# HKU-BAL/Clair3-RNA

Hardware: NVIDIA B200
Metric: candidate sites/sec (tensor+inference) (higher is better)
Workload: dtype int32 pileup + fp16/fp32-accumulate network

## Files before the change

clair3_rna_b200/build.py:

```python
import os
import subprocess
import sys

HERE = os.path.dirname(os.path.abspath(__file__))
CSRC = os.path.join(HERE, "csrc")
LIB = os.path.join(HERE, "libc3r_b200.so")
SOURCES = ["c3r_abi.cu", "bam_io.cpp", "decode.cpp", "fasta_io.cpp"]
HEADERS = ["scan.cuh", "pileup.cuh", "nn_fp32.cuh", "nn_tc.cuh", "nn_lstm2f.cuh", "tc_ptx.cuh", os.path.join("..", "..", "include", "c3r_b200.h")]
NVCC_FLAGS = ["-gencode", "arch=compute_100a,code=sm_100a", "-lineinfo", "-O3", "-std=c++17",
              "-Xcompiler", "-fPIC", "-shared", "-lcuda", "-lz", "-lpthread"]


def needs_build():
    if not os.path.exists(LIB):
        return True
    t = os.path.getmtime(LIB)
    return any(os.path.getmtime(os.path.join(CSRC, f)) > t for f in SOURCES + HEADERS)


def build(force=False, verbose=False):
    if not force and not needs_build():
        return LIB
    nvcc = os.environ.get("NVCC", "/usr/local/cuda/bin/nvcc")
    cmd = [nvcc] + NVCC_FLAGS + (["-Xptxas", "-v"] if verbose else []) + ["-o", LIB] + SOURCES
    out = subprocess.run(cmd, cwd=CSRC, stdout=subprocess.PIPE, stderr=subprocess.STDOUT, text=True)
    if out.returncode != 0:
        sys.stderr.write(out.stdout)
        raise RuntimeError("nvcc failed building libc3r_b200.so")
    if verbose:
        print(out.stdout)
    return LIB


if __name__ == "__main__":
    print(build(force="--force" in sys.argv, verbose="-v" in sys.argv))
```

clair3_rna_b200/csrc/nn_lstm2f.cuh:

```cuda
#pragma once

namespace c3r {

namespace ptx {
__device__ __forceinline__ void bulk_g2s_mcast(uint32_t dst, const void* src, uint32_t bytes, uint32_t bar, uint16_t mask) {
    asm volatile(
        "cp.async.bulk.shared::cluster.global.mbarrier::complete_tx::bytes.multicast::cluster [%0], [%1], %2, [%3], %4;"
        ::"r"(dst), "l"(src), "r"(bytes), "r"(bar), "h"(mask) : "memory");
}
}

constexpr int L2F_CH = 5;
constexpr int L2F_IMG = 8192;
constexpr int L2F_STAGES = 6;
constexpr int L2F_SLOT = 2 * L2F_IMG;
constexpr int L2F_LAST = 64 * 48 * 2;
constexpr int L2F_CHUNK_BYTES = 10 * L2F_IMG + L2F_LAST;
constexpr int L2F_STREAM_BYTES = L2F_CH * L2F_CHUNK_BYTES;
constexpr int L2F_NS = 4;
constexpr int L2F_GATE_WARPS = 16;
constexpr int L2F_THREADS = 128 + 32 * L2F_GATE_WARPS;
constexpr int L2F_AH = TC_TILE * U2 * 2;
constexpr int L2F_XB = TC_IMG * 2;
constexpr int L2F_OFF_X = 2 * L2F_AH;
// ... 173 lines not shown
            if (n_steps > 0)
                for (int kb = 0; kb < 4; ++kb) ptx::mbar_wait(b_xfree + 8 * kb, (n_steps - 1) & 1, a.err, 331);
        }
    } else if (warp == 2) {
        if (lane == 0) {
            const uint8_t* wsrc = a.wstream + ((size_t)dir * 2 + hr) * L2F_STREAM_BYTES;
            uint32_t wslot = 0, wph = 0, it = 0;
            long long pw[1] = {0};
            for (uint32_t g = 0; g < n_steps; ++g) {
                uint32_t off = 0;
                for (int cs = 0; cs < CH * L2F_STAGES; ++cs, ++it) {
                    const uint32_t bytes = (cs % L2F_STAGES) == L2F_STAGES - 1 ? L2F_LAST : L2F_SLOT;
                    L2F_WAIT(b_we + 8 * wslot, wph ^ 1, 340, 0);
                    ptx::mbar_arrive_expect_tx(b_wf + 8 * wslot, bytes);
                    if (NP == 1) ptx::bulk_g2s(s_W + wslot * L2F_SLOT, wsrc + off, bytes, b_wf + 8 * wslot);
                    else if (it % NP == pr) ptx::bulk_g2s_mcast(s_W + wslot * L2F_SLOT, wsrc + off, bytes, b_wf + 8 * wslot, mask_half);
                    off += bytes;
                    if (++wslot == L2F_NS) { wslot = 0; wph ^= 1; }
                }
            }
            if (PROF && pf) a.prof[8] = pw[0];
            const uint32_t total = n_steps * CH * L2F_STAGES;
            for (uint32_t k = total > (uint32_t)L2F_NS ? total - L2F_NS : 0; k < total; ++k)
                ptx::mbar_wait(b_we + 8 * (k % L2F_NS), (k / L2F_NS) & 1, a.err, 341);
        }
    } else if (warp == 3) {
        if (lane == 0 && hr == 1) {
            uint32_t wslot = 0, wph = 0;
            for (uint32_t g = 0; g < n_steps; ++g)
                for (int c = 0; c < CH; ++c)
                    for (int s = 0; s < L2F_STAGES; ++s) {
                        if (c == 0 && s < 4) {
                            ptx::mbar_wait(b_xf + 8 * s, g & 1, a.err, 350);
                            ptx::mbar_arrive_cluster_relaxed(b_xf + 8 * s, leader);
                        }
                        ptx::mbar_wait(b_wf + 8 * wslot, wph, a.err, 351);
                        ptx::mbar_arrive_cluster_relaxed(b_wf + 8 * wslot, leader);
                        if (++wslot == L2F_NS) { wslot = 0; wph ^= 1; }
                    }
        }
    } else {
        const int gw = warp - 4;
        const int q = warp & 3;
        const int sub = gw >> 2;
        const int row = q * 32 + lane;
        const uint32_t lane_addr = (uint32_t)(q * 32) << 16;
        uint32_t use = 0;
        const bool pfg = pf && gw == 0;
        long long pw[1] = {0};
        for (uint32_t g = 0; g < n_steps; ++g) {
            const int r = (int)(g / NT), step = (int)(g % NT);
            const int tp = j + r * J;
            const bool valid = tp < n_tile_pairs;
            const int tile = (valid ? tp : n_tile_pairs - 1) * 2 + (int)hr;
            const uint32_t nbuf = (g + 1) & 1;
            const int t = dir == 0 ? step : NT - 1 - step;
            uint8_t* ah = smem + nbuf * L2F_AH;
            __half* hout_t = a.hout + ((size_t)tile * NT + t) * 5 * TC_IMG;
            __half* hout_lo_t = a.hout_lo + ((size_t)tile * NT + t) * 5 * TC_IMG;
#pragma unroll
            for (int c = 0; c < CH; ++c, ++use) {
                const uint32_t slot = use & 1;
                if (PROF && pfg) { const long long t0 = clock64(); ptx::mbar_wait(b_accf + 8 * slot, (use >> 1) & 1, a.err, 308); pw[0] += clock64() - t0; }
                else ptx::mbar_wait(b_accf + 8 * slot, (use >> 1) & 1, a.err, 308);
                ptx::tc_fence_after();
                uint32_t cprev[8];
                uint32_t v[4][8];
#pragma unroll
                for (int gte = 0; gte < 4; ++gte) ptx::tmem_ld8(tmem + lane_addr + slot * 128 + gte * 32 + sub * 8, v[gte]);
                if (step > 0) ptx::tmem_ld8(tmem + lane_addr + C_COL + c * 32 + sub * 8, cprev);
                ptx::tmem_wait_ld();
                ptx::tc_fence_before();
                __syncwarp();
                if (lane == 0) ptx::mbar_arrive(b_acce + 8 * slot);
                uint32_t cnew[8];
                __align__(16) __half hh[8];
                __align__(16) __half hl[8];
#pragma unroll
                for (int u = 0; u < 8; ++u) {
                    const float zi = __uint_as_float(v[0][u]), zf = __uint_as_float(v[1][u]);
                    const float zg = __uint_as_float(v[2][u]), zo = __uint_as_float(v[3][u]);
                    const float cp = step > 0 ? __uint_as_float(cprev[u]) : 0.0f;
                    float cn, hv;
                    lstm_cell(zi, zf, zg, zo, cp, cn, hv);
                    cnew[u] = __float_as_uint(cn);
                    hh[u] = __float2half(hv);
                    hl[u] = __float2half(hv - __half2float(hh[u]));
                }
                ptx::tmem_st8(tmem + lane_addr + C_COL + c * 32 + sub * 8, cnew);
                const uint4 pk = *(const uint4*)hh;
                const int k8 = c * 4 + sub;
                *(uint4*)(ah + (size_t)k8 * (TC_TILE * 16) + row * 16) = pk;
                ptx::tmem_wait_st();
                if (c == CH - 1) {
                    ptx::tc_fence_before();
                    ptx::fence_proxy_async();
                    __syncwarp();
                    if (lane == 0) ptx::mbar_arrive(b_hrdy);
                }
                if (valid) {
                    const int col8 = (dir * U2) / 8 + k8;
                    const size_t oo = (size_t)(col8 / 8) * TC_IMG + (size_t)(col8 % 8) * (TC_TILE * 8) + row * 8;
                    *(uint4*)(hout_t + oo) = pk;
                    if (a.hout_lo) *(uint4*)(hout_lo_t + oo) = *(const uint4*)hl;
                }
            }
        }
        if (PROF && pfg && lane == 0) a.prof[9] = pw[0];
    }
    ptx::tc_fence_before();
    __syncthreads();
    ptx::cluster_sync();
    if (warp == 0) ptx::tmem_dealloc<2>(tmem, 512);
}

inline void lstm2f_pack(std::vector<uint8_t>& out, const float* h, size_t o_w2, size_t o_b2, size_t o_u2) {
    out.assign((size_t)4 * L2F_STREAM_BYTES, 0);
    auto split = [](float w, __half& hi, __half& lo) {
        hi = __float2half(w);
        lo = __float2half(w - __half2float(hi));
    };
    for (int dir = 0; dir < 2; ++dir)
        for (int hr = 0; hr < 2; ++hr) {
            __half* base = (__half*)(out.data() + ((size_t)dir * 2 + hr) * L2F_STREAM_BYTES);
            for (int c = 0; c < L2F_CH; ++c) {
                __half* ch = base + (size_t)c * (L2F_CHUNK_BYTES / 2);
                for (int jj = 0; jj < 64; ++jj) {
                    const int col = hr * 64 + jj, gate = col / 32, ul = col % 32;
                    const int kc = gate * U2 + c * 32 + ul;
                    const float gs = gate == 2 ? 1.0f : 0.5f;
                    for (int kb = 0; kb < 4; ++kb)
                        for (int k = 0; k < 64; ++k) {
                            __half hi, lo;
                            split(gs * h[o_w2 + (size_t)(kb * 64 + k) * 2 * G2 + dir * G2 + kc], hi, lo);
                            ch[(size_t)(2 * kb) * (L2F_IMG / 2) + ((size_t)(k / 8) * 64 * 8 + (size_t)jj * 8 + k % 8)] = hi;
                            ch[(size_t)(2 * kb + 1) * (L2F_IMG / 2) + ((size_t)(k / 8) * 64 * 8 + (size_t)jj * 8 + k % 8)] = lo;
                        }
                    for (int k = 0; k < U2; ++k) {
                        const int s = 8 + k / 64, kk = k % 64;
                        ch[(size_t)s * (L2F_IMG / 2) + ((size_t)(kk / 8) * 64 * 8 + (size_t)jj * 8 + kk % 8)] =
                            __float2half(gs * h[o_u2 + (size_t)dir * U2 * G2 + (size_t)k * G2 + kc]);
                    }
                    __half bh, bl;
                    split(gs * h[o_b2 + dir * G2 + kc], bh, bl);
                    __half* st10 = ch + (size_t)10 * (L2F_IMG / 2);
                    st10[(size_t)(32 / 8) * 64 * 8 + (size_t)jj * 8 + 0] = bh;
                    st10[(size_t)(32 / 8) * 64 * 8 + (size_t)jj * 8 + 1] = bl;
                }
            }
        }
}

template <int NP, bool PROF>
inline cudaError_t launch_lstm2f_np(const Lstm2fArgs& a, int sm_count, cudaStream_t st) {
    static bool attr = false;
    if (!attr) {
        cudaError_t e = cudaFuncSetAttribute(k_lstm2_fused<NP, PROF>, cudaFuncAttributeMaxDynamicSharedMemorySize, L2F_SMEM);
        if (e != cudaSuccess) return e;
        attr = true;
    }
    const int csize = 2 * NP;
    const int tile_pairs = a.n_tiles / 2;
    int per_dir = (tile_pairs + NP - 1) / NP;
    int max_per_dir = sm_count / csize / 2;
    if (NP > 1) {
        cudaLaunchConfig_t q = {};
        q.gridDim = dim3((unsigned)(sm_count / csize * csize)); q.blockDim = dim3(L2F_THREADS); q.dynamicSmemBytes = L2F_SMEM;
        cudaLaunchAttribute qa[1];
        qa[0].id = cudaLaunchAttributeClusterDimension;
        qa[0].val.clusterDim.x = csize; qa[0].val.clusterDim.y = 1; qa[0].val.clusterDim.z = 1;
        q.attrs = qa; q.numAttrs = 1;
        int n_cl = 0;
        if (cudaOccupancyMaxActiveClusters(&n_cl, k_lstm2_fused<NP, PROF>, &q) == cudaSuccess && n_cl > 0 && n_cl / 2 < max_per_dir)
            max_per_dir = n_cl / 2;
    }
    if (max_per_dir < 1) max_per_dir = 1;
    if (per_dir > max_per_dir) per_dir = max_per_dir;
    if (per_dir < 1) per_dir = 1;
    cudaLaunchConfig_t cfg = {};
    cfg.gridDim = dim3((unsigned)(per_dir * 2 * csize));
    cfg.blockDim = dim3(L2F_THREADS);
    cfg.dynamicSmemBytes = L2F_SMEM;
    cfg.stream = st;
    cudaLaunchAttribute at[1];
    at[0].id = cudaLaunchAttributeClusterDimension;
    at[0].val.clusterDim.x = csize; at[0].val.clusterDim.y = 1; at[0].val.clusterDim.z = 1;
    cfg.attrs = at; cfg.numAttrs = 1;
    return cudaLaunchKernelEx(&cfg, k_lstm2_fused<NP, PROF>, a);
}

inline int lstm2f_np() {
    static int v = -1;
    if (v < 0) {
        const char* e = getenv("C3R_LSTM2F_NP");
        v = e ? atoi(e) : 1;
        if (v != 1 && v != 2 && v != 4) v = 1;
    }
    return v;
}

inline cudaError_t launch_lstm2f(const Lstm2fArgs& a, int sm_count, cudaStream_t st) {
    if (a.prof) return launch_lstm2f_np<1, true>(a, sm_count, st);
    switch (lstm2f_np()) {
        case 2: return launch_lstm2f_np<2, false>(a, sm_count, st);
        case 4: return launch_lstm2f_np<4, false>(a, sm_count, st);
        default: return launch_lstm2f_np<1, false>(a, sm_count, st);
    }
}

}
```

clair3_rna_b200/csrc/nn_tc.cuh:

```cuda
#pragma once
#include <cstdint>
#include <cstdlib>
#include <string>
#include <vector>
#include <cuda_runtime.h>
#include <cuda_fp16.h>
#include "nn_fp32.cuh"
#include "tc_ptx.cuh"

namespace c3r {

constexpr int TC_TILE = 128;
constexpr int TC_KB = 64;
constexpr int TC_IMG = TC_TILE * TC_KB;
constexpr int lstm1_kx(int C) { return (3 * C + 2 + 15) / 16 * 16; }
constexpr int LSTM1_KX_MAX = lstm1_kx(30);

struct GemmArgs {
    const __half* A;
    const __half* B;
    const __half* A_lo;
    const __half* B_lo;
    int terms;
    const float* bias;
    float* out;
    int m_tiles, n_tiles, n_kb;
    int ksplit;
    size_t split_stride;
    int* err;
};

constexpr int GEMM_STAGES = 3;
constexpr int GEMM_THREADS = 192;
constexpr int GEMM_STAGE_BYTES = 4 * TC_IMG * 2;
constexpr int GEMM_SMEM = GEMM_STAGES * GEMM_STAGE_BYTES + 1024;

__global__ void __launch_bounds__(GEMM_THREADS, 1) k_gemm_tc(GemmArgs g) {
    extern __shared__ __align__(1024) uint8_t smem[];
    uint64_t* bars = (uint64_t*)(smem + GEMM_STAGES * GEMM_STAGE_BYTES);
    uint32_t* tmem_ptr_s = (uint32_t*)(bars + 12);
    float* bias_s = (float*)(bars + 32);
    const uint32_t s_base = ptx::smem_u32(smem);
    const uint32_t b_full = ptx::smem_u32(bars), b_empty = b_full + 32, b_accf = b_full + 64, b_acce = b_full + 80;
    const int warp = threadIdx.x >> 5, lane = threadIdx.x & 31;
    if (threadIdx.x == 0) {
        for (int i = 0; i < GEMM_STAGES; ++i) { ptx::mbar_init(b_full + 8 * i, 1); ptx::mbar_init(b_empty + 8 * i, 1); }
        for (int i = 0; i < 2; ++i) { ptx::mbar_init(b_accf + 8 * i, 1); ptx::mbar_init(b_acce + 8 * i, 4); }
        ptx::fence_barrier_init();
    }
    if (warp == 1) {
        ptx::tmem_alloc<1>(ptx::smem_u32(tmem_ptr_s), 256);
        ptx::tmem_relinquish<1>();
    }
    ptx::tc_fence_before();
    __syncthreads();
    ptx::tc_fence_after();
    const uint32_t tmem = *tmem_ptr_s;
    const int n_tiles_total = g.m_tiles * g.n_tiles;
    const int ksplit = g.ksplit > 1 ? g.ksplit : 1;
    const int n_items = n_tiles_total * ksplit;
    const uint32_t idesc = ptx::make_idesc_f16(128, 128);

    if (warp == 0) {
        if (lane == 0) {
            uint32_t it = 0;
            for (int item = blockIdx.x; item < n_items; item += gridDim.x) {
                const int tile = item % n_tiles_total, ks = item / n_tiles_total;
                const int m = tile / g.n_tiles, n = tile % g.n_tiles;
                const size_t ao = (size_t)m * g.n_kb * TC_IMG, bo = (size_t)n * g.n_kb * TC_IMG;
                const int kb0 = ks * g.n_kb / ksplit, kb1 = (ks + 1) * g.n_kb / ksplit;
                for (int kb = kb0; kb < kb1; ++kb, ++it) {
                    const uint32_t s = it % GEMM_STAGES, ph = (it / GEMM_STAGES) & 1;
                    const uint32_t dst = s_base + s * GEMM_STAGE_BYTES;
                    ptx::mbar_wait(b_empty + 8 * s, ph ^ 1, g.err, 101);
                    const bool a_lo = g.terms & 2;
                    ptx::mbar_arrive_expect_tx(b_full + 8 * s, a_lo ? GEMM_STAGE_BYTES : GEMM_STAGE_BYTES - TC_IMG * 2);
                    ptx::bulk_g2s(dst, g.A + ao + (size_t)kb * TC_IMG, TC_IMG * 2, b_full + 8 * s);
                    if (a_lo) ptx::bulk_g2s(dst + TC_IMG * 2, g.A_lo + ao + (size_t)kb * TC_IMG, TC_IMG * 2, b_full + 8 * s);
                    ptx::bulk_g2s(dst + 2 * TC_IMG * 2, g.B + bo + (size_t)kb * TC_IMG, TC_IMG * 2, b_full + 8 * s);
                    ptx::bulk_g2s(dst + 3 * TC_IMG * 2, g.B_lo + bo + (size_t)kb * TC_IMG, TC_IMG * 2, b_full + 8 * s);
                }
            }
        }
    } else if (warp == 1) {
        if (lane == 0) {
            uint32_t it = 0, tc = 0;
            for (int item = blockIdx.x; item < n_items; item += gridDim.x, ++tc) {
                const int ks = item / n_tiles_total;
                const int kb0 = ks * g.n_kb / ksplit, kb1 = (ks + 1) * g.n_kb / ksplit;
                const uint32_t slot = tc & 1, aph = (tc >> 1) & 1;
                ptx::mbar_wait(b_acce + 8 * slot, aph ^ 1, g.err, 102);
                ptx::tc_fence_after();
                for (int kb = kb0; kb < kb1; ++kb, ++it) {
                    const uint32_t s = it % GEMM_STAGES, ph = (it / GEMM_STAGES) & 1;
                    ptx::mbar_wait(b_full + 8 * s, ph, g.err, 103);
                    ptx::tc_fence_after();
                    const uint32_t st0 = s_base + s * GEMM_STAGE_BYTES;
#pragma unroll
                    for (int term = 0; term < 3; ++term) {
                        if (!((g.terms >> term) & 1)) continue;
                        const uint32_t sa = st0 + (term == 1 ? TC_IMG * 2 : 0), sb = st0 + (term == 2 ? 3 : 2) * TC_IMG * 2;
#pragma unroll
                        for (int k4 = 0; k4 < TC_KB / 16; ++k4) {
                            const uint64_t da = ptx::make_smem_desc(sa + k4 * 2 * (TC_TILE * 16), TC_TILE * 16, 128);
                            const uint64_t db = ptx::make_smem_desc(sb + k4 * 2 * (TC_TILE * 16), TC_TILE * 16, 128);
                            ptx::mma_f16<1>(tmem + slot * 128, da, db, idesc, (kb > kb0 || term > 0 || k4 > 0) ? 1u : 0u);
                        }
                    }
                    ptx::mma_commit_1(b_empty + 8 * s);
                }
                ptx::mma_commit_1(b_accf + 8 * slot);
            }
        }
    } else {
        const int q = warp & 3;
        const int row = q * 32 + lane;
        uint32_t tc = 0;
        for (int item = blockIdx.x; item < n_items; item += gridDim.x, ++tc) {
            const int tile = item % n_tiles_total, ks = item / n_tiles_total;
            const int m = tile / g.n_tiles, n = tile % g.n_tiles;
            const uint32_t slot = tc & 1, aph = (tc >> 1) & 1;
            ptx::mbar_wait(b_accf + 8 * slot, aph, g.err, 104);
            ptx::tc_fence_after();
            const uint32_t taddr = tmem + ((uint32_t)(q * 32) << 16) + slot * 128;
            asm volatile("bar.sync 1, 128;" ::: "memory");
            bias_s[threadIdx.x - 64] = g.bias[(size_t)n * 128 + (threadIdx.x - 64)];
            asm volatile("bar.sync 1, 128;" ::: "memory");
            const float* bias = bias_s;
#pragma unroll 1
            for (int j = 0; j < 8; ++j) {
                uint32_t v[16];
                ptx::tmem_ld16(taddr + j * 16, v);
                ptx::tmem_wait_ld();
                float* o = g.out + ((size_t)m * 128 + row) * ((size_t)g.n_tiles * 128) + (size_t)n * 128 + j * 16;
                if (ksplit > 1) {
                    float4* o4 = (float4*)(o + (size_t)ks * g.split_stride);
#pragma unroll
                    for (int c = 0; c < 4; ++c)
                        o4[c] = make_float4(__uint_as_float(v[4 * c]), __uint_as_float(v[4 * c + 1]), __uint_as_float(v[4 * c + 2]), __uint_as_float(v[4 * c + 3]));
                } else {
#pragma unroll
                    for (int c = 0; c < 16; ++c) o[c] = seluf_(__uint_as_float(v[c]) + bias[j * 16 + c]);
                }
            }
            ptx::tc_fence_before();
            __syncwarp();
            if (lane == 0) ptx::mbar_arrive(b_acce + 8 * slot);
        }
    }
    ptx::tc_fence_before();
    __syncthreads();
    if (warp == 1) ptx::tmem_dealloc<1>(tmem, 256);
}

template <int CH, int KX>
struct LstmCfg {
    static constexpr int U = CH * 32;
    static constexpr int KT = KX + U;
    static constexpr int B_BYTES = CH * 64 * KT * 2;
    static constexpr int AH_BYTES = TC_TILE * U * 2;
// ... 372 lines not shown
    void* abuf = nullptr;
    size_t abytes = 0;
    int cap_tiles = 0;
    __half* h1[2] = {};
    __half *h2 = nullptr, *h2_lo = nullptr, *xop = nullptr;
    __half* h1_cur = nullptr;
    float *l4 = nullptr, *l4p = nullptr;
    size_t l4_stride = 0;
    __half *l4h = nullptr, *l4h_lo = nullptr;
    float* a5 = nullptr;
    int* err = nullptr;
    long long* trace = nullptr;
    bool attr_set = false;
    struct TcPipe* pipe = nullptr;
};

inline void tc_pipe_release(struct TcPipe* p);
inline void tc_release(TcNet& t) {
    if (t.pipe) tc_pipe_release(t.pipe);
    if (t.wbuf) cudaFree(t.wbuf);
    if (t.abuf) cudaFree(t.abuf);
    if (t.err) cudaFree(t.err);
    if (t.trace) cudaFree(t.trace);
    t = TcNet();
}

inline size_t img_index(int R, int r, int k) { return (size_t)(k / 8) * R * 8 + (size_t)r * 8 + (k % 8); }

inline int tc_build(TcNet& t, const NetF32& net, const float* h, size_t o_w1, size_t o_b1, size_t o_u1, size_t o_w2,
                    size_t o_b2, size_t o_u2, size_t o_k4, size_t o_b4, size_t o_k51, size_t o_b51, size_t o_k52, size_t o_b52,
                    int sm_count, std::string* err) {
    tc_release(t);
    const int C = net.C;
    t.C = C;
    t.KX = lstm1_kx(C);
    t.sm_count = sm_count;
    const int KX = t.KX;
    const int KT1 = KX + U1;
    const size_t n_img1 = (size_t)2 * 2 * 4 * 64 * KT1;
    const size_t n_k4p = (size_t)(L4_IN / TC_KB) * TC_IMG;
    const size_t n_k5p = (size_t)2 * 2 * TC_IMG;
    std::vector<__half> hb(n_img1 + 2 * n_k4p + 2 * n_k5p);
    std::vector<float> fb(DENSE + 2 * DENSE);
    __half* img1 = hb.data();
    __half* k4p = img1 + n_img1;
    __half* k4p_lo = k4p + n_k4p;
    __half* k5p = k4p_lo + n_k4p;
    __half* k5p_lo = k5p + n_k5p;
    auto split = [](float w, __half& hi, __half& lo) {
        hi = __float2half(w);
        lo = __float2half(w - __half2float(hi));
    };
    for (int dir = 0; dir < 2; ++dir)
        for (int rank = 0; rank < 2; ++rank)
            for (int c = 0; c < 4; ++c) {
                __half* im = img1 + ((((size_t)dir * 2 + rank) * 4 + c) * 64) * KT1;
                for (int j = 0; j < 64; ++j) {
                    const int col = rank * 64 + j, gate = col / 32, ul = col % 32;
                    const int kc = gate * U1 + c * 32 + ul;
                    const float gs = gate == 2 ? 1.0f : 0.5f;
                    for (int k = 0; k < KT1; ++k) {
                        __half v = __float2half(0.0f);
                        if (k < 3 * C) {
                            const int ch = k % C;
                            __half hi, lo;
                            split(gs * h[o_w1 + (size_t)ch * 2 * G1 + dir * G1 + kc], hi, lo);
                            v = k >= C && k < 2 * C ? lo : hi;
                        } else if (k == 3 * C || k == 3 * C + 1) {
                            __half hi, lo;
                            split(gs * h[o_b1 + dir * G1 + kc], hi, lo);
                            v = k == 3 * C ? hi : lo;
                        } else if (k >= KX) {
                            v = __float2half(gs * h[o_u1 + (size_t)dir * U1 * G1 + (size_t)(k - KX) * G1 + kc]);
                        }
                        im[img_index(64, j, k)] = v;
                    }
                }
            }
    for (int k = 0; k < L4_IN; ++k)
        for (int j = 0; j < DENSE; ++j)
        {
            const size_t ix = (size_t)(k / TC_KB) * TC_IMG + img_index(128, j, k % TC_KB);
            split(h[o_k4 + (size_t)k * DENSE + j], k4p[ix], k4p_lo[ix]);
        }
    for (int j = 0; j < DENSE; ++j) fb[j] = h[o_b4 + j];
    for (int n = 0; n < 2; ++n)
        for (int k = 0; k < DENSE; ++k)
            for (int j = 0; j < DENSE; ++j) {
                const size_t ix = ((size_t)n * 2 + k / TC_KB) * TC_IMG + img_index(128, j, k % TC_KB);
                split(h[(n == 0 ? o_k51 : o_k52) + (size_t)k * DENSE + j], k5p[ix], k5p_lo[ix]);
            }
    for (int j = 0; j < DENSE; ++j) { fb[DENSE + j] = h[o_b51 + j]; fb[2 * DENSE + j] = h[o_b52 + j]; }

    std::vector<uint8_t> ws;
    lstm2f_pack(ws, h, o_w2, o_b2, o_u2);
    const size_t foff = ((hb.size() * 2 + 255) / 256) * 256;
    const size_t soff = ((foff + fb.size() * 4 + 1023) / 1024) * 1024;
    t.wbytes = soff + ws.size() + 256;
    cudaError_t e = cudaMalloc(&t.wbuf, t.wbytes);
    if (e != cudaSuccess) { *err = cudaGetErrorString(e); return -1; }
    uint8_t* d = (uint8_t*)t.wbuf;
    cudaMemcpy(d, hb.data(), hb.size() * 2, cudaMemcpyHostToDevice);
    cudaMemcpy(d + soff, ws.data(), ws.size(), cudaMemcpyHostToDevice);
    t.wstream2 = d + soff;
    e = cudaMemcpy(d + foff, fb.data(), fb.size() * 4, cudaMemcpyHostToDevice);
    if (e != cudaSuccess) { *err = cudaGetErrorString(e); return -1; }
    t.img1 = (const __half*)d;
    t.k4p = t.img1 + n_img1;
    t.k4p_lo = t.k4p + n_k4p;
    t.k5p = t.k4p_lo + n_k4p;
    t.k5p_lo = t.k5p + n_k5p;
    t.b4 = (const float*)(d + foff);
    t.b5p = t.b4 + DENSE;
    e = cudaMalloc((void**)&t.err, 64);
    if (e != cudaSuccess) { *err = cudaGetErrorString(e); return -1; }
    cudaMemset(t.err, 0, 64);
    if (getenv("C3R_TRACE")) {
        cudaMalloc((void**)&t.trace, 2 * 2 * NT * 8 * 8 * sizeof(long long));
        cudaMemset(t.trace, 0, 2 * 2 * NT * 8 * 8 * sizeof(long long));
    }
    t.ready = 1;
    return 0;
}

inline int tc_ensure(TcNet& t, int tiles, std::string* err) {
    if (tiles <= t.cap_tiles) return 0;
    if (t.abuf) cudaFree(t.abuf);
    t.abuf = nullptr;
    const size_t n_h1 = (size_t)tiles * NT * 4 * TC_IMG, n_h2 = (size_t)tiles * NT * 5 * TC_IMG;
    const size_t n_l4 = (size_t)tiles * 128 * DENSE;
    const size_t n_xop = (size_t)tiles * NT * LSTM1_KX_MAX * TC_TILE;
    t.abytes = (n_h1 + n_h2) * 2 * 2 + n_xop * 2 + n_l4 * (1 + L4_KSPLIT) * 4 + n_l4 * 2 * 2 + n_l4 * 2 * 4 + 1024;
    cudaError_t e = cudaMalloc(&t.abuf, t.abytes);
    if (e != cudaSuccess) { *err = std::string("activation scratch: ") + cudaGetErrorString(e); t.cap_tiles = 0; return -1; }
    uint8_t* p = (uint8_t*)t.abuf;
    t.l4 = (float*)p; p += n_l4 * 4;
    t.l4p = (float*)p; p += n_l4 * 4 * L4_KSPLIT;
    t.l4_stride = n_l4;
    t.a5 = (float*)p; p += n_l4 * 2 * 4;
    t.l4h = (__half*)p; p += n_l4 * 2;
    t.l4h_lo = (__half*)p; p += n_l4 * 2;
    t.h1[0] = (__half*)p; p += n_h1 * 2;
    t.h1[1] = (__half*)p; p += n_h1 * 2;
    t.h2 = (__half*)p; p += n_h2 * 2;
    t.h2_lo = (__half*)p; p += n_h2 * 2;
    t.xop = (__half*)p;
    t.cap_tiles = tiles;
    return 0;
}

constexpr int TC_SUB_TILES = 320;

template <int CH, int KX>
inline cudaError_t launch_lstm(const LstmArgs& a, int sm_count, cudaStream_t st) {
    typedef LstmCfg<CH, KX> Cfg;
    static bool attr = false;
    if (!attr) {
        cudaError_t e = cudaFuncSetAttribute(k_lstm_tc<CH, KX>, cudaFuncAttributeMaxDynamicSharedMemorySize, Cfg::SMEM);
        if (e != cudaSuccess) return e;
        attr = true;
    }
    int cpairs = a.n_tiles / 2;
    if (cpairs > sm_count / 4) cpairs = sm_count / 4;
    if (cpairs < 1) cpairs = 1;
    k_lstm_tc<CH, KX><<<cpairs * 4, LSTM_THREADS, Cfg::SMEM, st>>>(a);
    return cudaGetLastError();
}

inline int l4_terms() {
    static int v = -1;
    if (v < 0) {
        const char* e = getenv("C3R_L4_TERMS");
        v = e ? atoi(e) : 7;
        if (v < 1 || v > 7 || !(v & 1)) v = 7;
    }
    return v;
}

inline cudaError_t launch_gemm(const GemmArgs& g, int sm_count, cudaStream_t st) {
    static bool attr = false;
    if (!attr) {
        cudaError_t e = cudaFuncSetAttribute(k_gemm_tc, cudaFuncAttributeMaxDynamicSharedMemorySize, GEMM_SMEM);
        if (e != cudaSuccess) return e;
        attr = true;
    }
    int grid = g.m_tiles * g.n_tiles * (g.ksplit > 1 ? g.ksplit : 1);
    if (grid > sm_count) grid = sm_count;
    k_gemm_tc<<<grid, GEMM_THREADS, GEMM_SMEM, st>>>(g);
    return cudaGetLastError();
}

struct TcPipe {
    cudaStream_t s2 = nullptr;
    cudaEvent_t ev[2] = {};
    cudaEvent_t pass_done = nullptr;
    cudaEvent_t h1_free2[2] = {}, xop_free = nullptr, last_ready = nullptr, last_done = nullptr;
    int last_pairs = 0, parity = 0;
    long n_pass = 0, n_overlap = 0;
    bool ok = false;
};
inline int tc_pipe_init(TcPipe& p, std::string* err) {
    if (p.ok) return 0;
    int prio_lo = 0, prio_hi = 0;
    cudaDeviceGetStreamPriorityRange(&prio_lo, &prio_hi);
    cudaError_t e = cudaStreamCreateWithPriority(&p.s2, cudaStreamNonBlocking, getenv("C3R_FLAT_PRIORITY") ? prio_lo : prio_hi);
    for (int i = 0; i < 2 && e == cudaSuccess; ++i) e = cudaEventCreateWithFlags(&p.ev[i], cudaEventDisableTiming);
    if (e == cudaSuccess) e = cudaEventCreateWithFlags(&p.pass_done, cudaEventDisableTiming);
    for (cudaEvent_t* ev : {&p.h1_free2[0], &p.h1_free2[1], &p.xop_free, &p.last_ready, &p.last_done})
        if (e == cudaSuccess) e = cudaEventCreateWithFlags(ev, cudaEventDisableTiming);
    if (e != cudaSuccess) { *err = std::string("pipeline streams: ") + cudaGetErrorString(e); return -1; }
    p.ok = true;
    return 0;
}
inline void tc_pipe_release(TcPipe* p) {
    if (p->s2) cudaStreamDestroy(p->s2);
    for (cudaEvent_t e : p->ev) if (e) cudaEventDestroy(e);
    if (p->pass_done) cudaEventDestroy(p->pass_done);
    for (cudaEvent_t ev : {p->h1_free2[0], p->h1_free2[1], p->xop_free, p->last_ready, p->last_done}) if (ev) cudaEventDestroy(ev);
    delete p;
}

struct TcSub { int t0, nt; int64_t s0, ns; };

inline cudaError_t tc_lstm2(TcNet& t, const TcSub& b, cudaStream_t st, const __half* h1buf) {
    Lstm2fArgs f;
    f.wstream = t.wstream2; f.h1 = h1buf + (size_t)b.t0 * NT * 4 * TC_IMG;
    f.hout = t.h2 + (size_t)b.t0 * NT * 5 * TC_IMG;
    f.hout_lo = (l4_terms() & 2) ? t.h2_lo + (size_t)b.t0 * NT * 5 * TC_IMG : nullptr;
    f.n_tiles = b.nt; f.err = t.err;
    f.prof = (t.trace && b.t0 == 0) ? t.trace + 2 * NT * 8 * 8 : nullptr;
    return launch_lstm2f(f, t.sm_count, st);
}
inline cudaError_t tc_l4_heads(TcNet& t, const NetF32& net, const TcSub& b, float* probs, cudaStream_t st) {
    GemmArgs g4;
    g4.A = t.h2 + (size_t)b.t0 * NT * 5 * TC_IMG; g4.B = t.k4p; g4.A_lo = t.h2_lo + (size_t)b.t0 * NT * 5 * TC_IMG; g4.B_lo = t.k4p_lo;
    g4.terms = l4_terms(); g4.bias = t.b4; g4.out = t.l4p + (size_t)b.t0 * 128 * DENSE; g4.m_tiles = b.nt; g4.n_tiles = 1; g4.n_kb = L4_IN / TC_KB;
    g4.ksplit = L4_KSPLIT; g4.split_stride = t.l4_stride; g4.err = t.err;
    cudaError_t e = launch_gemm(g4, t.sm_count, st);
    if (e != cudaSuccess) return e;
    k_l4_finish<<<b.nt * 4, 128, 0, st>>>(t.l4p + (size_t)b.t0 * 128 * DENSE, L4_KSPLIT, t.l4_stride, t.b4,
                                      t.l4 + (size_t)b.t0 * 128 * DENSE, t.l4h + (size_t)b.t0 * 2 * TC_IMG, t.l4h_lo + (size_t)b.t0 * 2 * TC_IMG);
    GemmArgs g5;
    g5.A = t.l4h + (size_t)b.t0 * 2 * TC_IMG; g5.A_lo = t.l4h_lo + (size_t)b.t0 * 2 * TC_IMG; g5.B = t.k5p; g5.B_lo = t.k5p_lo;
    g5.terms = 7; g5.bias = t.b5p; g5.out = t.a5 + (size_t)b.t0 * 128 * 256; g5.m_tiles = b.nt; g5.n_tiles = 2; g5.n_kb = 2;
    g5.ksplit = 1; g5.split_stride = 0; g5.err = t.err;
    e = launch_gemm(g5, t.sm_count, st);
    if (e != cudaSuccess) return e;
    {
        int64_t blocks = (b.ns + HOUT_WARPS - 1) / HOUT_WARPS;
        if (blocks > (int64_t)t.sm_count * 4) blocks = (int64_t)t.sm_count * 4;
        if (blocks > 0) k_heads_out<<<(unsigned)blocks, HOUT_WARPS * 32, 0, st>>>(net, t.a5 + (size_t)b.t0 * 128 * 256, probs + b.s0 * 24, b.ns);
    }
    return cudaGetLastError();
}

inline int tc_forward(TcNet& t, const NetF32& net, const int32_t* tensor, int64_t n, float* probs, cudaStream_t st,
                      std::string* err, const __half* xop_ready = nullptr) {
    if (!t.ready) { *err = "weights not packed"; return -1; }
    if (!t.pipe) t.pipe = new TcPipe();
    if (tc_pipe_init(*t.pipe, err)) return -1;
    TcPipe& P = *t.pipe;
    int launches = 0;
#define TCK(call, what) do { cudaError_t e__ = (call); if (e__ != cudaSuccess) { *err = std::string(what) + ": " + cudaGetErrorString(e__); return -1; } } while (0)
    const int round_tiles = 2 * (t.sm_count / 4) > 0 ? 2 * (t.sm_count / 4) : 2;
    const int sub_tiles = TC_SUB_TILES >= round_tiles ? (TC_SUB_TILES / round_tiles) * round_tiles : TC_SUB_TILES;
    for (int64_t o = 0; o < n; o += (int64_t)sub_tiles * TC_TILE) {
        const int64_t m = n - o < (int64_t)sub_tiles * TC_TILE ? n - o : (int64_t)sub_tiles * TC_TILE;
        int tiles = (int)((m + TC_TILE - 1) / TC_TILE);
        tiles += tiles & 1;
        if (tc_ensure(t, tiles, err)) return -1;
        const int hb = P.parity;
        P.parity ^= 1;
        __half* const h1buf = t.h1[hb];
        t.h1_cur = h1buf;
        TCK(cudaStreamWaitEvent(st, P.h1_free2[hb], 0), "wait");
        if (!xop_ready) TCK(cudaStreamWaitEvent(st, P.xop_free, 0), "wait");
        const __half* xop_in = t.xop;
        if (xop_ready) xop_in = xop_ready + (size_t)(o / TC_TILE) * NT * (size_t)(t.KX * TC_TILE);
        else {
            if (t.C == 18) k_xop<18, lstm1_kx(18)><<<tiles * NT, TC_TILE, 0, st>>>(tensor + o * NT * t.C, t.xop, m);
            else k_xop<30, lstm1_kx(30)><<<tiles * NT, TC_TILE, 0, st>>>(tensor + o * NT * t.C, t.xop, m);
            ++launches;
        }
        const int pairs = tiles / 2;
        const int per_round = (t.sm_count / (2 * lstm2f_np()) / 2) * lstm2f_np();
        int pa = pairs;
        if (pairs > per_round && pairs % per_round != 0) pa = (pairs / per_round) * per_round;
        TcSub A, B;
        A.t0 = 0; A.nt = 2 * pa; A.s0 = 0; A.ns = m < (int64_t)A.nt * TC_TILE ? m : (int64_t)A.nt * TC_TILE;
        B.t0 = A.nt; B.nt = tiles - A.nt; B.s0 = A.ns; B.ns = m - A.ns;
        auto lstm1 = [&](const TcSub& b, cudaStream_t s) -> cudaError_t {
            LstmArgs a1;
            a1.Wimg = t.img1; a1.xop = xop_in + (size_t)b.t0 * NT * t.KX * TC_TILE;
            a1.hout = h1buf + (size_t)b.t0 * NT * 4 * TC_IMG;
            a1.n_sites = b.ns; a1.n_tiles = b.nt; a1.err = t.err; a1.trace = b.t0 == 0 ? t.trace : nullptr;
            return t.C == 18 ? launch_lstm<4, lstm1_kx(18)>(a1, t.sm_count, s) : launch_lstm<4, lstm1_kx(30)>(a1, t.sm_count, s);
        };
        const int ip = (t.sm_count - 4 * P.last_pairs) / 4;
        bool overlap = o == 0 && P.last_pairs > 0 && ip >= 8 && getenv("C3R_NO_LSTM1_OVERLAP") == nullptr;
        if (overlap) {
            overlap = cudaEventQuery(P.last_done) == cudaErrorNotReady;
            (void)cudaGetLastError();
        }
        auto piece = [&](int p0, int np) {
            TcSub b; b.t0 = 2 * p0; b.nt = 2 * np; b.s0 = (int64_t)b.t0 * TC_TILE;
            const int64_t left = m - b.s0;
            b.ns = left < 0 ? 0 : left < (int64_t)b.nt * TC_TILE ? left : (int64_t)b.nt * TC_TILE;
            return b;
        };
        ++P.n_pass;
        if (overlap) {
            ++P.n_overlap;
            TCK(cudaStreamWaitEvent(st, P.last_ready, 0), "wait");
            int done = 0;
            for (int c = 0; c < 2 && done < pairs; ++c) {
                const int np = pairs - done < ip ? pairs - done : ip;
                TCK(lstm1(piece(done, np), st), "lstm1");
                done += np; ++launches;
            }
            if (done < pairs) {
                TCK(cudaStreamWaitEvent(st, P.last_done, 0), "wait");
                TCK(lstm1(piece(done, pairs - done), st), "lstm1");
            } else --launches;
        } else {
            TcSub all; all.t0 = 0; all.nt = tiles; all.s0 = 0; all.ns = m;
            TCK(lstm1(all, st), "lstm1");
        }
        TCK(cudaEventRecord(P.xop_free, st), "event");
        TCK(cudaStreamWaitEvent(st, P.pass_done, 0), "wait");
        ++launches;
        float* pr = probs + o * 24;
        if (B.nt == 0) TCK(cudaEventRecord(P.last_ready, st), "event");
        TCK(tc_lstm2(t, A, st, h1buf), "lstm2");
        ++launches;
        if (B.nt == 0) {
            TCK(cudaEventRecord(P.last_done, st), "event");
            TCK(cudaEventRecord(P.h1_free2[hb], st), "event");
            P.last_pairs = pa;
            TCK(tc_l4_heads(t, net, A, pr, st), "l4/heads");
            launches += 4;
            TCK(cudaEventRecord(P.pass_done, st), "event");
            continue;
        }
        TCK(cudaEventRecord(P.ev[0], st), "event");
        TCK(cudaEventRecord(P.last_ready, st), "event");
        TCK(tc_lstm2(t, B, st, h1buf), "lstm2");
        TCK(cudaEventRecord(P.last_done, st), "event");
        TCK(cudaEventRecord(P.h1_free2[hb], st), "event");
        P.last_pairs = B.nt / 2;
        TCK(cudaStreamWaitEvent(P.s2, P.ev[0], 0), "wait");
        TCK(tc_l4_heads(t, net, A, pr, P.s2), "l4/heads");
        TCK(cudaEventRecord(P.ev[1], P.s2), "event");
        TCK(tc_l4_heads(t, net, B, pr, st), "l4/heads");
        TCK(cudaStreamWaitEvent(st, P.ev[1], 0), "wait");
        launches += 9;
        TCK(cudaEventRecord(P.pass_done, st), "event");
    }
#undef TCK
    return launches;
}

inline int tc_check_error(TcNet& t, cudaStream_t st, int* code) {
    int h[1] = {0};
    if (!t.err) { *code = 0; return 0; }
    cudaError_t e = cudaMemcpyAsync(h, t.err, 4, cudaMemcpyDeviceToHost, st);
    if (e == cudaSuccess) e = cudaStreamSynchronize(st);
    if (e != cudaSuccess) return -1;
    *code = h[0];
    if (h[0]) cudaMemsetAsync(t.err, 0, 4, st);
    return 0;
}

}
```

Measured before the change: 10.14 million.

## Add cost-model pass scheduler splitting LSTM stages across two streams

Introduces a small cost model (fixed per-round times for LSTM1, LSTM2 and tail) that searches for a two-group split of SM slots. When the pair count is not a multiple of the round size, one group runs LSTM1 then LSTM2 while the other is still working, so ragged remainder rounds are meant to overlap across two streams instead of serialising. Launch helpers gain caps on grid size, and event dependencies are generalised to follow the plan. It adds more events and waits, and relies on hardcoded timing constants that may not match real kernel times.

```diff
diff --git a/clair3_rna_b200/build.py b/clair3_rna_b200/build.py
--- a/clair3_rna_b200/build.py
+++ b/clair3_rna_b200/build.py
@@ -6,7 +6,7 @@
 CSRC = os.path.join(HERE, "csrc")
 LIB = os.path.join(HERE, "libc3r_b200.so")
 SOURCES = ["c3r_abi.cu", "bam_io.cpp", "decode.cpp", "fasta_io.cpp"]
-HEADERS = ["scan.cuh", "pileup.cuh", "nn_fp32.cuh", "nn_tc.cuh", "nn_lstm2f.cuh", "tc_ptx.cuh", os.path.join("..", "..", "include", "c3r_b200.h")]
+HEADERS = ["scan.cuh", "pileup.cuh", "nn_fp32.cuh", "nn_tc.cuh", "nn_lstm2f.cuh", "nn_sched.h", "tc_ptx.cuh", os.path.join("..", "..", "include", "c3r_b200.h")]
 NVCC_FLAGS = ["-gencode", "arch=compute_100a,code=sm_100a", "-lineinfo", "-O3", "-std=c++17",
               "-Xcompiler", "-fPIC", "-shared", "-lcuda", "-lz", "-lpthread"]
 
diff --git a/clair3_rna_b200/csrc/nn_lstm2f.cuh b/clair3_rna_b200/csrc/nn_lstm2f.cuh
--- a/clair3_rna_b200/csrc/nn_lstm2f.cuh
+++ b/clair3_rna_b200/csrc/nn_lstm2f.cuh
@@ -349,7 +349,7 @@
 }
 
 template <int NP, bool PROF>
-inline cudaError_t launch_lstm2f_np(const Lstm2fArgs& a, int sm_count, cudaStream_t st) {
+inline cudaError_t launch_lstm2f_np(const Lstm2fArgs& a, int sm_count, int max_clusters, cudaStream_t st) {
     static bool attr = false;
     if (!attr) {
         cudaError_t e = cudaFuncSetAttribute(k_lstm2_fused<NP, PROF>, cudaFuncAttributeMaxDynamicSharedMemorySize, L2F_SMEM);
@@ -371,6 +371,7 @@
         if (cudaOccupancyMaxActiveClusters(&n_cl, k_lstm2_fused<NP, PROF>, &q) == cudaSuccess && n_cl > 0 && n_cl / 2 < max_per_dir)
             max_per_dir = n_cl / 2;
     }
+    if (max_per_dir > max_clusters) max_per_dir = max_clusters;
     if (max_per_dir < 1) max_per_dir = 1;
     if (per_dir > max_per_dir) per_dir = max_per_dir;
     if (per_dir < 1) per_dir = 1;
@@ -396,13 +397,13 @@
     return v;
 }
 
-inline cudaError_t launch_lstm2f(const Lstm2fArgs& a, int sm_count, cudaStream_t st) {
-    if (a.prof) return launch_lstm2f_np<1, true>(a, sm_count, st);
+inline cudaError_t launch_lstm2f(const Lstm2fArgs& a, int sm_count, int max_clusters, cudaStream_t st) {
+    if (a.prof) return launch_lstm2f_np<1, true>(a, sm_count, max_clusters, st);
     switch (lstm2f_np()) {
-        case 2: return launch_lstm2f_np<2, false>(a, sm_count, st);
-        case 4: return launch_lstm2f_np<4, false>(a, sm_count, st);
-        default: return launch_lstm2f_np<1, false>(a, sm_count, st);
-    }
-}
-
-}
+        case 2: return launch_lstm2f_np<2, false>(a, sm_count, max_clusters, st);
+        case 4: return launch_lstm2f_np<4, false>(a, sm_count, max_clusters, st);
+        default: return launch_lstm2f_np<1, false>(a, sm_count, max_clusters, st);
+    }
+}
+
+}
diff --git a/clair3_rna_b200/csrc/nn_sched.h b/clair3_rna_b200/csrc/nn_sched.h
--- /dev/null
+++ b/clair3_rna_b200/csrc/nn_sched.h
@@ -0,0 +1,102 @@
+#pragma once
+
+namespace c3r {
+
+constexpr int SCHED_T_LSTM1 = 144;
+constexpr int SCHED_T_LSTM2 = 365;
+constexpr int SCHED_T_TAIL = 100;
+
+enum SchedKind { SCHED_LSTM1 = 0, SCHED_LSTM2 = 1, SCHED_L4H = 2 };
+
+struct SchedLaunch {
+    int stream;
+    int kind;
+    int p0, np;
+    int cap;
+    int wait;
+};
+
+struct SchedPlan {
+    int n = 0;
+    SchedLaunch l[8];
+    int split = 0;
+    int t_model = 0;
+};
+
+inline int sched_ceil(int a, int b) { return (a + b - 1) / b; }
+inline int sched_max(int a, int b) { return a > b ? a : b; }
+
+inline void sched_add(SchedPlan& p, int stream, int kind, int p0, int np, int cap, int wait) {
+    SchedLaunch& l = p.l[p.n++];
+    l.stream = stream; l.kind = kind; l.p0 = p0; l.np = np; l.cap = cap; l.wait = wait;
+}
+
+inline SchedPlan sched_rounds(int P, int S, int lstm2_round) {
+    SchedPlan p;
+    const int pa = P > lstm2_round && P % lstm2_round != 0 ? (P / lstm2_round) * lstm2_round : P;
+    sched_add(p, 0, SCHED_LSTM1, 0, P, S, -1);
+    sched_add(p, 0, SCHED_LSTM2, 0, pa, lstm2_round, -1);
+    const int t_a = sched_ceil(P, S) * SCHED_T_LSTM1 + sched_ceil(pa, lstm2_round) * SCHED_T_LSTM2;
+    if (pa == P) {
+        sched_add(p, 0, SCHED_L4H, 0, P, 0, -1);
+        p.t_model = t_a + sched_ceil(P, S) * SCHED_T_TAIL;
+        return p;
+    }
+    sched_add(p, 0, SCHED_LSTM2, pa, P - pa, lstm2_round, -1);
+    sched_add(p, 1, SCHED_L4H, 0, pa, 0, 1);
+    sched_add(p, 0, SCHED_L4H, pa, P - pa, 0, -1);
+    p.t_model = sched_max(t_a + sched_ceil(pa, S) * SCHED_T_TAIL, t_a + SCHED_T_LSTM2 + sched_ceil(P - pa, S) * SCHED_T_TAIL);
+    return p;
+}
+
+inline int sched_two_group_time(int P, int S, int sx, int ny, int* x_last) {
+    const int sy = S - sx, n2 = P - sx - ny;
+    const int ty1 = sched_ceil(P - sx, sy) * SCHED_T_LSTM1;
+    const int ty2 = ty1 + (ny ? sched_ceil(ny, sy) * SCHED_T_LSTM2 : 0);
+    const int tx1 = SCHED_T_LSTM1 + SCHED_T_LSTM2;
+    const int tx2 = n2 ? sched_max(tx1, ty1) + sched_ceil(n2, sx) * SCHED_T_LSTM2 : tx1;
+    *x_last = tx2 >= ty2;
+    if (n2 == 0)
+        return sched_max(tx1 + sched_ceil(sx, S) * SCHED_T_TAIL, ty2 + sched_ceil(ny, S) * SCHED_T_TAIL);
+    if (!*x_last) return -1;
+    return sched_max(sched_max(ty2, tx1) + sched_ceil(sx + ny, S) * SCHED_T_TAIL, tx2 + sched_ceil(n2, S) * SCHED_T_TAIL);
+}
+
+inline SchedPlan sched_plan(int P, int S, int lstm2_round, int lstm2_np) {
+    SchedPlan best = sched_rounds(P, S, lstm2_round);
+    if (lstm2_np != 1 || lstm2_round != S || S < 2 || P <= S || P % S == 0) return best;
+    int bt = best.t_model, bsx = 0, bny = 0, bx = 0;
+    for (int sx = 1; sx < S; ++sx)
+        for (int ny = 0; ny <= P - sx; ++ny) {
+            int x_last = 0;
+            const int t = sched_two_group_time(P, S, sx, ny, &x_last);
+            if (t >= 0 && t < bt) { bt = t; bsx = sx; bny = ny; bx = x_last; }
+        }
+    if (bsx == 0) return best;
+    const int sx = bsx, sy = S - sx, ny = bny, n2 = P - sx - ny;
+    SchedPlan p;
+    p.split = 1;
+    p.t_model = bt;
+    sched_add(p, 0, SCHED_LSTM1, 0, sx, sx, -1);
+    sched_add(p, 1, SCHED_LSTM1, sx, P - sx, sy, -1);
+    if (n2 > 0) {
+        sched_add(p, 0, SCHED_LSTM2, 0, sx, sx, -1);
+        if (ny) sched_add(p, 1, SCHED_LSTM2, sx, ny, sy, -1);
+        sched_add(p, 0, SCHED_LSTM2, sx + ny, n2, sx, 1);
+        sched_add(p, 1, SCHED_L4H, 0, sx + ny, 0, 2);
+        sched_add(p, 0, SCHED_L4H, sx + ny, n2, 0, -1);
+    } else if (bx) {
+        sched_add(p, 1, SCHED_LSTM2, sx, ny, sy, -1);
+        sched_add(p, 0, SCHED_LSTM2, 0, sx, sx, -1);
+        sched_add(p, 1, SCHED_L4H, sx, ny, 0, -1);
+        sched_add(p, 0, SCHED_L4H, 0, sx, 0, -1);
+    } else {
+        sched_add(p, 0, SCHED_LSTM2, 0, sx, sx, -1);
+        sched_add(p, 1, SCHED_LSTM2, sx, ny, sy, -1);
+        sched_add(p, 0, SCHED_L4H, 0, sx, 0, -1);
+        sched_add(p, 1, SCHED_L4H, sx, ny, 0, -1);
+    }
+    return p;
+}
+
+}
diff --git a/clair3_rna_b200/csrc/nn_tc.cuh b/clair3_rna_b200/csrc/nn_tc.cuh
--- a/clair3_rna_b200/csrc/nn_tc.cuh
+++ b/clair3_rna_b200/csrc/nn_tc.cuh
@@ -1,11 +1,13 @@
 #pragma once
 #include <cstdint>
 #include <cstdlib>
+#include <cstring>
 #include <string>
 #include <vector>
 #include <cuda_runtime.h>
 #include <cuda_fp16.h>
 #include "nn_fp32.cuh"
+#include "nn_sched.h"
 #include "tc_ptx.cuh"
 
 namespace c3r {
@@ -684,7 +686,7 @@
 constexpr int TC_SUB_TILES = 320;
 
 template <int CH, int KX>
-inline cudaError_t launch_lstm(const LstmArgs& a, int sm_count, cudaStream_t st) {
+inline cudaError_t launch_lstm(const LstmArgs& a, int sm_count, int max_cpairs, cudaStream_t st) {
     typedef LstmCfg<CH, KX> Cfg;
     static bool attr = false;
     if (!attr) {
@@ -694,6 +696,7 @@
     }
     int cpairs = a.n_tiles / 2;
     if (cpairs > sm_count / 4) cpairs = sm_count / 4;
+    if (cpairs > max_cpairs) cpairs = max_cpairs;
     if (cpairs < 1) cpairs = 1;
     k_lstm_tc<CH, KX><<<cpairs * 4, LSTM_THREADS, Cfg::SMEM, st>>>(a);
     return cudaGetLastError();
@@ -724,10 +727,12 @@
 
 struct TcPipe {
     cudaStream_t s2 = nullptr;
-    cudaEvent_t ev[2] = {};
+    cudaEvent_t ev[8] = {};
+    cudaEvent_t fork = nullptr;
     cudaEvent_t pass_done = nullptr;
     cudaEvent_t h1_free2[2] = {}, xop_free = nullptr, last_ready = nullptr, last_done = nullptr;
     int last_pairs = 0, parity = 0;
+    bool last_split = false;
     long n_pass = 0, n_overlap = 0;
     bool ok = false;
 };
@@ -736,7 +741,8 @@
     int prio_lo = 0, prio_hi = 0;
     cudaDeviceGetStreamPriorityRange(&prio_lo, &prio_hi);
     cudaError_t e = cudaStreamCreateWithPriority(&p.s2, cudaStreamNonBlocking, getenv("C3R_FLAT_PRIORITY") ? prio_lo : prio_hi);
-    for (int i = 0; i < 2 && e == cudaSuccess; ++i) e = cudaEventCreateWithFlags(&p.ev[i], cudaEventDisableTiming);
+    for (int i = 0; i < 8 && e == cudaSuccess; ++i) e = cudaEventCreateWithFlags(&p.ev[i], cudaEventDisableTiming);
+    if (e == cudaSuccess) e = cudaEventCreateWithFlags(&p.fork, cudaEventDisableTiming);
     if (e == cudaSuccess) e = cudaEventCreateWithFlags(&p.pass_done, cudaEventDisableTiming);
     for (cudaEvent_t* ev : {&p.h1_free2[0], &p.h1_free2[1], &p.xop_free, &p.last_ready, &p.last_done})
         if (e == cudaSuccess) e = cudaEventCreateWithFlags(ev, cudaEventDisableTiming);
@@ -747,6 +753,7 @@
 inline void tc_pipe_release(TcPipe* p) {
     if (p->s2) cudaStreamDestroy(p->s2);
     for (cudaEvent_t e : p->ev) if (e) cudaEventDestroy(e);
+    if (p->fork) cudaEventDestroy(p->fork);
     if (p->pass_done) cudaEventDestroy(p->pass_done);
     for (cudaEvent_t ev : {p->h1_free2[0], p->h1_free2[1], p->xop_free, p->last_ready, p->last_done}) if (ev) cudaEventDestroy(ev);
     delete p;
@@ -754,14 +761,14 @@
 
 struct TcSub { int t0, nt; int64_t s0, ns; };
 
-inline cudaError_t tc_lstm2(TcNet& t, const TcSub& b, cudaStream_t st, const __half* h1buf) {
+inline cudaError_t tc_lstm2(TcNet& t, const TcSub& b, int max_pairs, cudaStream_t st, const __half* h1buf) {
     Lstm2fArgs f;
     f.wstream = t.wstream2; f.h1 = h1buf + (size_t)b.t0 * NT * 4 * TC_IMG;
     f.hout = t.h2 + (size_t)b.t0 * NT * 5 * TC_IMG;
     f.hout_lo = (l4_terms() & 2) ? t.h2_lo + (size_t)b.t0 * NT * 5 * TC_IMG : nullptr;
     f.n_tiles = b.nt; f.err = t.err;
     f.prof = (t.trace && b.t0 == 0) ? t.trace + 2 * NT * 8 * 8 : nullptr;
-    return launch_lstm2f(f, t.sm_count, st);
+    return launch_lstm2f(f, t.sm_count, max_pairs / lstm2f_np(), st);
 }
 inline cudaError_t tc_l4_heads(TcNet& t, const NetF32& net, const TcSub& b, float* probs, cudaStream_t st) {
     GemmArgs g4;
@@ -815,18 +822,14 @@
             ++launches;
         }
         const int pairs = tiles / 2;
+        const int slots = t.sm_count / 4 > 0 ? t.sm_count / 4 : 1;
         const int per_round = (t.sm_count / (2 * lstm2f_np()) / 2) * lstm2f_np();
-        int pa = pairs;
-        if (pairs > per_round && pairs % per_round != 0) pa = (pairs / per_round) * per_round;
-        TcSub A, B;
-        A.t0 = 0; A.nt = 2 * pa; A.s0 = 0; A.ns = m < (int64_t)A.nt * TC_TILE ? m : (int64_t)A.nt * TC_TILE;
-        B.t0 = A.nt; B.nt = tiles - A.nt; B.s0 = A.ns; B.ns = m - A.ns;
-        auto lstm1 = [&](const TcSub& b, cudaStream_t s) -> cudaError_t {
+        auto lstm1 = [&](const TcSub& b, int cap, cudaStream_t s) -> cudaError_t {
             LstmArgs a1;
             a1.Wimg = t.img1; a1.xop = xop_in + (size_t)b.t0 * NT * t.KX * TC_TILE;
             a1.hout = h1buf + (size_t)b.t0 * NT * 4 * TC_IMG;
             a1.n_sites = b.ns; a1.n_tiles = b.nt; a1.err = t.err; a1.trace = b.t0 == 0 ? t.trace : nullptr;
-            return t.C == 18 ? launch_lstm<4, lstm1_kx(18)>(a1, t.sm_count, s) : launch_lstm<4, lstm1_kx(30)>(a1, t.sm_count, s);
+            return t.C == 18 ? launch_lstm<4, lstm1_kx(18)>(a1, t.sm_count, cap, s) : launch_lstm<4, lstm1_kx(30)>(a1, t.sm_count, cap, s);
         };
         const int ip = (t.sm_count - 4 * P.last_pairs) / 4;
         bool overlap = o == 0 && P.last_pairs > 0 && ip >= 8 && getenv("C3R_NO_LSTM1_OVERLAP") == nullptr;
@@ -840,52 +843,80 @@
             b.ns = left < 0 ? 0 : left < (int64_t)b.nt * TC_TILE ? left : (int64_t)b.nt * TC_TILE;
             return b;
         };
+        const char* ps = getenv("C3R_PASS_SCHEDULE");
+        const SchedPlan plan = overlap || (ps && strcmp(ps, "rounds") == 0) ? sched_rounds(pairs, slots, per_round)
+                                                                            : sched_plan(pairs, slots, per_round, lstm2f_np());
         ++P.n_pass;
+        int first = 0;
         if (overlap) {
             ++P.n_overlap;
             TCK(cudaStreamWaitEvent(st, P.last_ready, 0), "wait");
-            int done = 0;
-            for (int c = 0; c < 2 && done < pairs; ++c) {
-                const int np = pairs - done < ip ? pairs - done : ip;
-                TCK(lstm1(piece(done, np), st), "lstm1");
-                done += np; ++launches;
-            }
-            if (done < pairs) {
-                TCK(cudaStreamWaitEvent(st, P.last_done, 0), "wait");
-                TCK(lstm1(piece(done, pairs - done), st), "lstm1");
-            } else --launches;
-        } else {
-            TcSub all; all.t0 = 0; all.nt = tiles; all.s0 = 0; all.ns = m;
-            TCK(lstm1(all, st), "lstm1");
-        }
-        TCK(cudaEventRecord(P.xop_free, st), "event");
-        TCK(cudaStreamWaitEvent(st, P.pass_done, 0), "wait");
-        ++launches;
+            if (P.last_split) {
+                TCK(lstm1(piece(0, pairs), slots, st), "lstm1");
+            } else {
+                int done = 0;
+                for (int c = 0; c < 2 && done < pairs; ++c) {
+                    const int np = pairs - done < ip ? pairs - done : ip;
+                    TCK(lstm1(piece(done, np), slots, st), "lstm1");
+                    done += np; ++launches;
+                }
+                if (done < pairs) {
+                    TCK(cudaStreamWaitEvent(st, P.last_done, 0), "wait");
+                    TCK(lstm1(piece(done, pairs - done), slots, st), "lstm1");
+                } else --launches;
+            }
+            TCK(cudaEventRecord(P.ev[0], st), "event");
+            first = 1;
+            ++launches;
+        }
+        cudaStream_t ss[2] = {st, P.s2};
+        TCK(cudaEventRecord(P.fork, st), "event");
+        TCK(cudaStreamWaitEvent(P.s2, P.fork, 0), "wait");
+        auto last_of = [&](int kind, int s, int i) {
+            int r = -1;
+            for (int j = 0; j < i; ++j) if (plan.l[j].kind == kind && plan.l[j].stream == s) r = j;
+            return r;
+        };
+        int l1_last = -1, l2_last = -1, l2_prev = -1, s2_last = -1;
+        for (int i = 0; i < plan.n; ++i) {
+            if (plan.l[i].kind == SCHED_LSTM1) l1_last = i;
+            if (plan.l[i].kind == SCHED_LSTM2) { l2_prev = l2_last; l2_last = i; }
+            if (plan.l[i].stream == 1) s2_last = i;
+        }
+        bool h2_free[2] = {false, false};
         float* pr = probs + o * 24;
-        if (B.nt == 0) TCK(cudaEventRecord(P.last_ready, st), "event");
-        TCK(tc_lstm2(t, A, st, h1buf), "lstm2");
-        ++launches;
-        if (B.nt == 0) {
-            TCK(cudaEventRecord(P.last_done, st), "event");
-            TCK(cudaEventRecord(P.h1_free2[hb], st), "event");
-            P.last_pairs = pa;
-            TCK(tc_l4_heads(t, net, A, pr, st), "l4/heads");
-            launches += 4;
-            TCK(cudaEventRecord(P.pass_done, st), "event");
-            continue;
-        }
-        TCK(cudaEventRecord(P.ev[0], st), "event");
-        TCK(cudaEventRecord(P.last_ready, st), "event");
-        TCK(tc_lstm2(t, B, st, h1buf), "lstm2");
-        TCK(cudaEventRecord(P.last_done, st), "event");
-        TCK(cudaEventRecord(P.h1_free2[hb], st), "event");
-        P.last_pairs = B.nt / 2;
-        TCK(cudaStreamWaitEvent(P.s2, P.ev[0], 0), "wait");
-        TCK(tc_l4_heads(t, net, A, pr, P.s2), "l4/heads");
-        TCK(cudaEventRecord(P.ev[1], P.s2), "event");
-        TCK(tc_l4_heads(t, net, B, pr, st), "l4/heads");
-        TCK(cudaStreamWaitEvent(st, P.ev[1], 0), "wait");
-        launches += 9;
+        for (int i = 0; i < plan.n; ++i) {
+            const SchedLaunch& L = plan.l[i];
+            cudaStream_t s = ss[L.stream];
+            const int other = L.stream ^ 1;
+            if (L.wait >= 0) TCK(cudaStreamWaitEvent(s, P.ev[L.wait], 0), "wait");
+            if (L.kind == SCHED_LSTM2 && !h2_free[L.stream]) {
+                TCK(cudaStreamWaitEvent(s, P.pass_done, 0), "wait");
+                h2_free[L.stream] = true;
+            }
+            if (i == l2_last && l2_prev < 0) TCK(cudaEventRecord(P.last_ready, s), "event");
+            if (i >= first) {
+                if (L.kind == SCHED_LSTM1) TCK(lstm1(piece(L.p0, L.np), L.cap, s), "lstm1");
+                else if (L.kind == SCHED_LSTM2) TCK(tc_lstm2(t, piece(L.p0, L.np), L.cap, s, h1buf), "lstm2");
+                else { TCK(tc_l4_heads(t, net, piece(L.p0, L.np), pr, s), "l4/heads"); launches += 3; }
+                ++launches;
+                TCK(cudaEventRecord(P.ev[i], s), "event");
+            }
+            const int kind_last = i == l1_last ? SCHED_LSTM1 : i == l2_last || i == l2_prev ? SCHED_LSTM2 : -1;
+            if (kind_last >= 0) {
+                const int j = last_of(kind_last, other, i);
+                if (j >= 0) TCK(cudaStreamWaitEvent(s, P.ev[j], 0), "wait");
+            }
+            if (i == l1_last) TCK(cudaEventRecord(P.xop_free, s), "event");
+            if (i == l2_prev) TCK(cudaEventRecord(P.last_ready, s), "event");
+            if (i == l2_last) {
+                TCK(cudaEventRecord(P.last_done, s), "event");
+                TCK(cudaEventRecord(P.h1_free2[hb], s), "event");
+                P.last_pairs = L.np < L.cap ? L.np : L.cap;
+                P.last_split = plan.split != 0;
+            }
+        }
+        if (s2_last >= 0) TCK(cudaStreamWaitEvent(st, P.ev[s2_last], 0), "wait");
         TCK(cudaEventRecord(P.pass_done, st), "event");
     }
 #undef TCK
```

After: 10.79 million (median of 6 runs). +6.4%, better.
